# Kiteretsu77/This_and_That_VDM

Hardware: AMD Instinct MI355X
Metric: denoise-steps/sec (14-frame 256x448 VGL, 25 steps) (higher is better)
Workload: dtype bf16; 1 GPU; VGL denoise step: GestureNet ControlNet + spatio-temporal UNet + per-frame CFG + Euler, latent 14x4x32x56, CFG batch 2, 78 context tokens, heads (5,10,20,20); mode=vgl, requests_per_gpu=1, parallelism=1 independent request(s), one per GPU; RCCL weight broadcast at start-up only, hipgraph=True, finite_output=True, spatial_self_attention=bf16, weights_identical_on_all_ranks=True

## Files before the change

### this_and_that_vdm_amd/csrc/attention.hip

```cpp
#include <stdlib.h>
#include <type_traits>
#include "common.h"

#ifndef TT_ATTN_PIPE_SGB
#define TT_ATTN_PIPE_SGB 1
#endif

namespace {

struct AttnP {
  const char* q; long ldq;
  const char* k; long ldk;
  const char* vt; long ldvt;
  char* out; long ldo;
  int nseq, lq, heads;
  int mask, lk, k_seq_stride, v_seq_stride, frames, ctx_batches, batch0;
  int k_rows_total;
  long vt_cols_total;
  unsigned k_bytes, vt_bytes;
  float scale_log2e;
  const char* qx; long ldqx; const char* wq; long ldwq; const float* bq; int qc; float ln_eps;
  unsigned qx_bytes, wq_bytes;
  int v_rows;
};

constexpr int QB = 128;
constexpr int KB = 64;

__device__ __forceinline__ float fast_exp2(float x) { return __builtin_amdgcn_exp2f(x); }

struct Bid3 { int x, y, z; };
#ifndef TT_ATTN_QP_HEADFAST
#define TT_ATTN_QP_HEADFAST 1
#endif
template <bool HEADFAST = false>
__device__ __forceinline__ Bid3 xcd_remap3() {
  const int gx = gridDim.x, gy = gridDim.y;
  const int nwg = gx * gy * (int)gridDim.z;
  int bid = (int)blockIdx.x + gx * ((int)blockIdx.y + gy * (int)blockIdx.z);
  const int q = nwg >> 3, r = nwg & 7, xcd = bid & 7, idx = bid >> 3;
  bid = (xcd < r ? xcd * (q + 1) : r * (q + 1) + (xcd - r) * q) + idx;
  Bid3 o;
  if constexpr (HEADFAST) {
    o.y = bid % gy;
    const int t = bid / gy;
    o.x = t % gx;
    o.z = t / gx;
  } else {
    o.x = bid % gx;
    const int t = bid / gx;
    o.y = t % gy;
    o.z = t / gy;
  }
  return o;
}


__device__ __forceinline__ int key_perm(int l31) { return 16 * ((l31 >> 2) & 1) + (l31 & 3) + 4 * (l31 >> 3); }

template <int QES, int D>
__device__ __forceinline__ void load_q_frags(const AttnP& p, int seq, int head, int qrow, bool qok, int hi, uint4 (&qf)[D * QES / 32]) {
  const char* qp = p.q + (((long)seq * p.lq + (qok ? qrow : 0)) * p.ldq + head * D) * QES;
#pragma unroll
  for (int n = 0; n < D * QES / 32; ++n) qf[n] = qok ? *(const uint4*)(qp + (n * 2 + hi) * 16) : make_uint4(0, 0, 0, 0);
}

__device__ __forceinline__ void vr_read_addrs(int lane, unsigned lds_base, unsigned (&out)[2]) {
  const int gi = lane & 15, gg = lane >> 4, r2 = gi >> 2;
  const int base = ((gg & 1) * 2 + ((gi & 3) >> 1)) ^ ((gi >> 3) & 1);
#pragma unroll
  for (int half = 0; half < 2; ++half)
    out[half] = lds_base + (gg >> 1) * 2048 + r2 * 128 + half * 512 + ((base ^ (half << 1)) << 4) + (gi & 1) * 8;
}

template <int EB, int D, bool VR, int DH = D>
struct KvStage {
  static constexpr int EPC = 16 / EB;
  static constexpr int KCPR = D / EPC, VCPR = VR ? D / EPC : KB / EPC;
  static_assert(DH <= D && DH % EPC == 0, "whole chunks of the head");
  static constexpr int K_BYTES = KB * D * EB, V_BYTES = D * KB * EB, STAGE = K_BYTES + V_BYTES;
  static constexpr int KPT = (KB * KCPR) / 256, VPT = ((VR ? KB : D) * VCPR) / 256;
  static_assert(KPT * 4096 == K_BYTES && VPT * 4096 == V_BYTES, "the staged pieces cover each tile exactly");
  static constexpr int INV = (int)0x80000000;
  static_assert(KPT >= 1 && VPT >= 1, "tile smaller than the block");
  const AttnP& p;
  char* const ring;
  const __amdgpu_buffer_rsrc_t rk, rv;
  int kvo[KPT], kr[KPT], vvo[VPT], vc[VPT];
  const int k_rows_left;
  const long v_cols_left;
  __device__ __forceinline__ KvStage(const AttnP& p_, char* smem, int tid, int wid, int head, int kbase, int vbase)
      : p(p_), ring(smem + wid * 1024),
        rk(__builtin_amdgcn_make_buffer_rsrc((void*)p_.k, 0, p_.k_bytes, 0x00020000)),
        rv(__builtin_amdgcn_make_buffer_rsrc((void*)p_.vt, 0, p_.vt_bytes, 0x00020000)),
        k_rows_left(p_.k_rows_total - kbase), v_cols_left(p_.vt_cols_total - vbase) {
#pragma unroll
    for (int i = 0; i < KPT; ++i) {
      const int slot = i * 256 + tid;
      const int r = slot / KCPR, c = (slot % KCPR) ^ tile_swz<KCPR>(r);
      kr[i] = r;
      kvo[i] = (int)((((long)kbase + r) * p.ldk + head * DH + c * EPC) * EB);
      if (DH != D && c * EPC >= DH) kvo[i] = INV;
    }
#pragma unroll
    for (int i = 0; i < VPT; ++i) {
      const int slot = i * 256 + tid;
      const int r = slot / VCPR, c = (slot % VCPR) ^ tile_swz<VCPR>(r);
      if constexpr (VR) {
        vc[i] = r;
        vvo[i] = (int)((((long)vbase + r) * p.ldvt + head * DH + c * EPC) * EB);
        if (DH != D && c * EPC >= DH) vvo[i] = INV;
      } else {
        vc[i] = c * EPC;
        vvo[i] = (int)(((long)(head * DH + r) * p.ldvt + vbase + c * EPC) * EB);
        if (DH != D && r >= DH) vvo[i] = INV;
      }
    }
  }
  __device__ __forceinline__ void stage(int buf, int tile) const {
    const int j0 = tile * KB;
    char* lk_ = ring + buf * STAGE;
    char* lv_ = ring + buf * STAGE + K_BYTES;
    const int soff_k = __builtin_amdgcn_readfirstlane((int)((long)j0 * p.ldk * EB));
    const int soff_v = VR ? __builtin_amdgcn_readfirstlane((int)((long)j0 * p.ldvt * EB)) : j0 * EB;
    const bool edge = j0 + KB > k_rows_left || j0 + KB > v_cols_left;
#pragma unroll
    for (int i = 0; i < KPT; ++i) {
      int v = kvo[i];
      if (edge && j0 + kr[i] >= k_rows_left) v = INV;
      __builtin_amdgcn_raw_ptr_buffer_load_lds(rk, (__attribute__((address_space(3))) void*)(lk_ + i * 4096), 16, v, soff_k, 0, 0);
    }
#pragma unroll
    for (int i = 0; i < VPT; ++i) {
      int v = vvo[i];
      if (edge && j0 + vc[i] >= v_cols_left) v = INV;
      __builtin_amdgcn_raw_ptr_buffer_load_lds(rv, (__attribute__((address_space(3))) void*)(lv_ + i * 4096), 16, v, soff_v, 0, 0);
    }
  }
};

template <typename F>
__device__ __forceinline__ void for_each_tile(int ntiles, int lk, F&& tile) {
  const bool ragged = (lk % KB) != 0;
  const int full = ragged ? ntiles - 1 : ntiles;
  int t = 0;
  for (; t + 1 < full; t += 2) {
    tile(t, std::integral_constant<int, 0>{}, std::false_type{});
    tile(t + 1, std::integral_constant<int, 1>{}, std::false_type{});
  }
  if (t < full) {
    tile(t, std::integral_constant<int, 0>{}, std::false_type{});
    if (ragged) tile(t + 1, std::integral_constant<int, 1>{}, std::true_type{});
  } else if (ragged) {
    tile(t, std::integral_constant<int, 0>{}, std::true_type{});
  }
}

__device__ __forceinline__ void mask_ragged(f32x16_t (&s)[2], int t, int hi, int lk) {
  const int j0 = t * KB;
#pragma unroll
  for (int kb = 0; kb < 2; ++kb)
#pragma unroll
    for (int r = 0; r < 16; ++r) {
      const int j = j0 + kb * 32 + hi * 16 + r;
      if (j >= lk) s[kb][r] = -INFINITY;
    }
}

template <int NO, bool WITH_OX = false>
__device__ __forceinline__ void softmax_rescale(const f32x16_t (&s)[2], float scale_log2e, float& m_run, float& l_run, f32x16_t (&o)[NO],
                                                f32x16_t* ox = nullptr) {
  float mx = s[0][0];
#pragma unroll
  for (int kb = 0; kb < 2; ++kb)
#pragma unroll
    for (int r = 0; r < 16; ++r) mx = fmaxf(mx, s[kb][r]);
  mx = fmaxf(mx, __shfl_xor(mx, 32));
  const float m_new = fmaxf(m_run, mx * scale_log2e);
  const float alpha = fast_exp2(m_run - m_new);
  l_run *= alpha;
#pragma unroll
  for (int i = 0; i < NO; ++i)
#pragma unroll
    for (int r = 0; r < 16; ++r) { o[i][r] *= alpha; if constexpr (WITH_OX) ox[i][r] *= alpha; }
  m_run = m_new;
}

template <typename Tag, int D, int DO = D, int NO = D / 32>
__device__ __forceinline__ void attn_store_rows(const AttnP& p, char* smem, const f32x16_t (&o)[NO], float l_run, int wid, int lane,
                                                int seq, int head, int qblk, int qstride, int qcls) {
  static_assert(NO * 32 >= DO && NO * 32 <= D && (DO * Elem<Tag>::ES) % 16 == 0, "accumulators cover the stored columns");
  typedef typename Elem<Tag>::quad_t quad_t;
  constexpr int ES = Elem<Tag>::ES;
  const int l31 = lane & 31, hi = lane >> 5;
  const float l_tot = l_run + __shfl_xor(l_run, 32);
  const float inv = l_tot > 0.f ? 1.0f / l_tot : 0.f;
  __syncthreads();
  constexpr int ROWB_O = D * ES, CPR_O = ROWB_O / 16;
  char* strip = smem + wid * (32 * ROWB_O);
#pragma unroll
  for (int db = 0; db < NO; ++db)
#pragma unroll
    for (int g = 0; g < 4; ++g) {
      const int byte = (db * 32 + 8 * g + 4 * hi) * ES;
      const float v4[4] = {o[db][g * 4] * inv, o[db][g * 4 + 1] * inv, o[db][g * 4 + 2] * inv, o[db][g * 4 + 3] * inv};
      *(quad_t*)(strip + l31 * ROWB_O + (((byte >> 4) ^ (l31 & (CPR_O - 1))) << 4) + (byte & 15)) = f32_to_quad<Tag>(v4);
    }
  constexpr int RPP = 64 / CPR_O;
  const int oc = lane % CPR_O, orow = lane / CPR_O;
#pragma unroll
  for (int pass = 0; pass < 32 / RPP; ++pass) {
    const int r = pass * RPP + orow;
    const uint4 v = *(const uint4*)(strip + r * ROWB_O + ((oc ^ (r & (CPR_O - 1))) << 4));
    const int qr = (qblk * QB + wid * 32 + r) * qstride + qcls;
    if (qr < p.lq && (DO == D || oc * 16 < DO * ES)) *(uint4*)(p.out + (((long)seq * p.lq + qr) * p.ldo + head * DO) * ES + oc * 16) = v;
  }
}

template <typename Tag, int D, int MASK, bool QP = false, bool VR = false, bool SP = false>
__global__ __launch_bounds__(256, (D == 64 && Elem<Tag>::ES == 2) ? 2 : 1) void attn_kernel(const AttnP p) {
  static_assert(!VR || (D == 64 && Elem<Tag>::ES == 2 && MASK == 0 && !QP), "row-major V: spatial self-attention, head dimension 64, 16-bit storage");
  static_assert(!SP || (Elem<Tag>::ES == 4 && !QP && !VR), "split products: the fp32-storage kernel");
  kernarg_touch<sizeof(AttnP)>();
  extern __shared__ __attribute__((aligned(16))) char smem[];
  constexpr int ES = Elem<Tag>::ES, EPC = Elem<Tag>::EPC;
  typedef KvStage<ES, D, VR> Stage;
  constexpr int KCPR = Stage::KCPR, VCPR = Stage::VCPR, K_BYTES = Stage::K_BYTES, STAGE = Stage::STAGE;
  constexpr int DS = KCPR / 2, DB = D / 32;
  constexpr int PH = 16 / EPC;

  const int tid = threadIdx.x, lane = tid & 63;
  const int wid = __builtin_amdgcn_readfirstlane(tid >> 6);
  const int l31 = lane & 31, hi = lane >> 5;
  const Bid3 blk = xcd_remap3<QP && TT_ATTN_QP_HEADFAST>();
  const int head = blk.y, seq = blk.z;
  const char* zero = (const char*)tt_zero_page;

  const int qstride = MASK == 2 ? p.ctx_batches : 1;
  const int qcls = MASK == 2 ? blk.x % qstride : 0;
  const int qblk = MASK == 2 ? blk.x / qstride : blk.x;
  int kbase, vbase;
  if (MASK == 0) { kbase = seq * p.k_seq_stride; vbase = seq * p.v_seq_stride; }
  else {
    const int b = p.batch0 + seq / p.frames;
    const int ctx = MASK == 1 ? b : (int)(((long)b * p.lq + qcls) % p.ctx_batches);
    kbase = ctx * p.k_seq_stride; vbase = ctx * p.v_seq_stride;
  }
  const int ntiles = (p.lk + KB - 1) / KB;

  const int qrow = (qblk * QB + wid * 32 + l31) * qstride + qcls;
  const bool qok = qrow < p.lq;
  uint4 qf[DS];
  if constexpr (!QP) {
    load_q_frags<ES, D>(p, seq, head, qrow, qok, hi, qf);
  } else {
    static_assert(!QP || (D == 64 && ES == 2 && MASK != 0), "fused query projection: cross-attention, head dimension 64, 16-bit storage");
    constexpr int QSLAB = QB * 128 + 64 * 128, QNST = 3;
    constexpr int QINV = (int)0x80000000;
    const __amdgpu_buffer_rsrc_t rx = __builtin_amdgcn_make_buffer_rsrc((void*)p.qx, 0, p.qx_bytes, 0x00020000);
    const __amdgpu_buffer_rsrc_t rwq = __builtin_amdgcn_make_buffer_rsrc((void*)p.wq, 0, p.wq_bytes, 0x00020000);
    int xo[4], wo[2];
#pragma unroll
    for (int i = 0; i < 4; ++i) {
      const int slot = i * 256 + tid, r = slot >> 3, c = (slot & 7) ^ tile_swz<8>(r);
      const int qr = (qblk * QB + r) * qstride + qcls;
      xo[i] = qr < p.lq ? (int)((((long)seq * p.lq + qr) * p.ldqx + c * 8) * 2) : QINV;
    }
#pragma unroll
    for (int i = 0; i < 2; ++i) {
      const int slot = i * 256 + tid, r = slot >> 3, c = (slot & 7) ^ tile_swz<8>(r);
      wo[i] = (int)((((long)head * 64 + r) * p.ldwq + c * 8) * 2);
    }
    const int nslab = p.qc >> 6;
    auto qstage = [&](int s) {
      char* dst = smem + (s % QNST) * QSLAB + wid * 1024;
      const int soff = __builtin_amdgcn_readfirstlane(s * 128);
      const bool ok = s < nslab;
#pragma unroll
      for (int i = 0; i < 4; ++i)
        __builtin_amdgcn_raw_ptr_buffer_load_lds(rx, (__attribute__((address_space(3))) void*)(dst + i * 4096), 16, ok ? xo[i] : QINV, soff, 0, 0);
#pragma unroll
      for (int i = 0; i < 2; ++i)
        __builtin_amdgcn_raw_ptr_buffer_load_lds(rwq, (__attribute__((address_space(3))) void*)(dst + QB * 128 + i * 4096), 16, ok ? wo[i] : QINV, soff, 0, 0);
    };
    f32x16_t qa[2];
#pragma unroll
    for (int j = 0; j < 2; ++j)
#pragma unroll
      for (int r = 0; r < 16; ++r) qa[j][r] = 0.f;
    float ls = 0.f, lq2 = 0.f;
    const unsigned qbase = lds_addr(smem);
    const int xr = wid * 32 + l31;
    unsigned xa[4], wa[4];
#pragma unroll
    for (int ks = 0; ks < 4; ++ks) {
      xa[ks] = tile_off<8>(xr, ks * 2 + hi);
      wa[ks] = QB * 128 + tile_off<8>(l31, ks * 2 + hi);
    }
    qstage(0); qstage(1);
    for (int s = 0; s < nslab; ++s) {
      asm volatile("s_waitcnt vmcnt(6)" ::: "memory");
      __syncthreads();
      qstage(s + 2);
      const unsigned sb = qbase + (s % QNST) * QSLAB;
      raw_u32x4_t xf[4], wf[2][4];
#pragma unroll
      for (int ks = 0; ks < 4; ++ks) {
        xf[ks] = lds_read16_raw(sb + xa[ks]);
        wf[0][ks] = lds_read16_raw(sb + wa[ks]);
        wf[1][ks] = lds_read16_raw_off<4096>(sb + wa[ks]);
      }
      lds_wait<0>();
#pragma unroll
      for (int ks = 0; ks < 4; ++ks) {
        ln_stat<Tag>(xf[ks], ls, lq2);
#pragma unroll
        for (int j = 0; j < 2; ++j)
          qa[j] = Cvt<Tag>::mfma32(make_uint4(wf[j][ks].x, wf[j][ks].y, wf[j][ks].z, wf[j][ks].w),
                                   make_uint4(xf[ks].x, xf[ks].y, xf[ks].z, xf[ks].w), qa[j]);
      }
      __builtin_amdgcn_sched_barrier(0);
    }
    asm volatile("s_waitcnt vmcnt(0)" ::: "memory");
    __syncthreads();
    const float inv_c = 1.0f / (float)p.qc;
    const float sm = (ls + __shfl_xor(ls, 32)) * inv_c, sq = (lq2 + __shfl_xor(lq2, 32)) * inv_c;
    const float rs = rsqrtf(fmaxf(sq - sm * sm, 0.f) + p.ln_eps);
#pragma unroll
    for (int ds = 0; ds < DS; ++ds) {
      const int j = ds >> 1, t = ds & 1;
      const float4 b0 = *(const float4*)(p.bq + head * 64 + 32 * j + 8 * (2 * t) + 4 * hi);
      const float4 b1 = *(const float4*)(p.bq + head * 64 + 32 * j + 8 * (2 * t + 1) + 4 * hi);
      const float v[8] = {fmaf(qa[j][(2 * t) * 4], rs, b0.x), fmaf(qa[j][(2 * t) * 4 + 1], rs, b0.y), fmaf(qa[j][(2 * t) * 4 + 2], rs, b0.z),
                          fmaf(qa[j][(2 * t) * 4 + 3], rs, b0.w), fmaf(qa[j][(2 * t + 1) * 4], rs, b1.x), fmaf(qa[j][(2 * t + 1) * 4 + 1], rs, b1.y),
                          fmaf(qa[j][(2 * t + 1) * 4 + 2], rs, b1.z), fmaf(qa[j][(2 * t + 1) * 4 + 3], rs, b1.w)};
      qf[ds] = qok ? pack8<Tag>(v) : make_uint4(0, 0, 0, 0);
    }
  }

  const Stage kv(p, smem, tid, wid, head, kbase, vbase);

  f32x16_t o[DB];
#pragma unroll
  for (int i = 0; i < DB; ++i)
#pragma unroll
    for (int r = 0; r < 16; ++r) o[i][r] = 0.f;
  float m_run = -1e30f, l_run = 0.f;
  f32x16_t ox[SP ? DB : 1];
  uint4 qh[SP ? DS / 2 : 1], ql[SP ? DS / 2 : 1];
  if constexpr (SP) {
#pragma unroll
    for (int i = 0; i < DB; ++i)
#pragma unroll
      for (int r = 0; r < 16; ++r) ox[i][r] = 0.f;
#pragma unroll
    for (int i = 0; i < DS / 2; ++i) {
      uint2 h0, l0, h1, l1;
      split_f16x4(qf[2 * i].x, qf[2 * i].y, qf[2 * i].z, qf[2 * i].w, h0, l0);
      split_f16x4(qf[2 * i + 1].x, qf[2 * i + 1].y, qf[2 * i + 1].z, qf[2 * i + 1].w, h1, l1);
      qh[i] = make_uint4(h0.x, h0.y, h1.x, h1.y); ql[i] = make_uint4(l0.x, l0.y, l1.x, l1.y);
    }
  }

  const int pi = key_perm(l31);

  const unsigned lds_base = lds_addr(smem);
  constexpr bool PRE = D == 64 && ES == 2;
  unsigned kaddr[PRE ? 2 : 1][PRE ? DS : 1], vaddr[PRE ? DB : 1][PRE ? 2 * PH : 1];
  if constexpr (PRE) {
#pragma unroll
    for (int kb = 0; kb < 2; ++kb)
#pragma unroll
      for (int ds = 0; ds < DS; ++ds) kaddr[kb][ds] = lds_base + tile_off<KCPR>(kb * 32 + pi, ds * 2 + hi);
#pragma unroll
    for (int db = 0; db < DB; ++db)
#pragma unroll
      for (int k = 0; k < 2 * PH; ++k) vaddr[db][k] = lds_base + tile_off<VCPR>(db * 32 + l31, (k / PH) * (32 / EPC) + hi * PH + k % PH);
  }
  unsigned vr_addr[2] = {0u, 0u};
  if constexpr (VR) vr_read_addrs(lane, lds_base, vr_addr);
  auto k_addr = [&](int kb, int ds) -> unsigned {
    if constexpr (PRE) return kaddr[kb][ds]; else return lds_base + tile_off<KCPR>(kb * 32 + pi, ds * 2 + hi);
  };
  auto v_addr = [&](int db, int k) -> unsigned {
    if constexpr (PRE) return vaddr[db][k]; else return lds_base + tile_off<VCPR>(db * 32 + l31, (k / PH) * (32 / EPC) + hi * PH + k % PH);
  };

  constexpr int NBK = DS / 2;
  constexpr int NBV = (DB / 2) * PH;
  static_assert(DS % 2 == 0 && DB % 2 == 0, "fragment batches of four");
  auto tile = [&](int t, auto buf_tag, auto mask_tag) {
    constexpr int BUF = decltype(buf_tag)::value;
    constexpr bool MASKED = decltype(mask_tag)::value;
    constexpr int KOFF = BUF * STAGE, VOFF = BUF * STAGE + K_BYTES;
    asm volatile("s_waitcnt vmcnt(0)" ::: "memory");
    __syncthreads();
    if (t + 1 < ntiles) kv.stage(BUF ^ 1, t + 1);
    raw_u32x4_t fa[4], fb[4];
    auto read_k = [&](int i, raw_u32x4_t (&f)[4]) {
#pragma unroll
      for (int j = 0; j < 4; ++j) f[j] = lds_read16_raw_off<KOFF>(k_addr(j & 1, 2 * i + (j >> 1)));
    };
    auto read_v = [&](int i, raw_u32x4_t (&f)[4]) {
#pragma unroll
      for (int j = 0; j < 4; ++j) f[j] = lds_read16_raw_off<VOFF>(v_addr(2 * (i / PH) + (j & 1), 2 * (i % PH) + (j >> 1)));
    };
    raw_u32x2_t ga[8], gb[8];
    auto read_vr = [&](auto i_tag, raw_u32x2_t (&f)[8]) {
      constexpr int I = decltype(i_tag)::value;
      auto one = [&](auto j_tag) {
        constexpr int J = decltype(j_tag)::value;
        constexpr int db = 2 * (I / PH) + (J & 1), k = 2 * (I % PH) + (J >> 1), kb = k / PH, h = k % PH;
        constexpr int off = VOFF + kb * 4096 + h * 1024 + ((db ^ h) << 6);
        f[2 * J] = lds_read8_tr_off<off>(vr_addr[0]);
        f[2 * J + 1] = lds_read8_tr_off<off>(vr_addr[1]);
      };
      one(std::integral_constant<int, 0>{}); one(std::integral_constant<int, 1>{});
      one(std::integral_constant<int, 2>{}); one(std::integral_constant<int, 3>{});
    };
    f32x16_t s[2], sx[SP ? 2 : 1];
#pragma unroll
    for (int kb = 0; kb < 2; ++kb)
#pragma unroll
      for (int r = 0; r < 16; ++r) { s[kb][r] = 0.f; if constexpr (SP) sx[kb][r] = 0.f; }
    read_k(0, fa);
    read_k(1, fb);
#pragma unroll
    for (int i = 0; i < NBK; ++i) {
      if (i + 1 < NBK) lds_wait<4>(); else lds_wait<0>();
      const raw_u32x4_t (&f)[4] = (i & 1) ? fb : fa;
      if constexpr (SP) {
#pragma unroll
        for (int kb = 0; kb < 2; ++kb) {
          uint2 h0, l0, h1, l1;
          split_f16x4(f[kb].x, f[kb].y, f[kb].z, f[kb].w, h0, l0);
          split_f16x4(f[kb + 2].x, f[kb + 2].y, f[kb + 2].z, f[kb + 2].w, h1, l1);
          const uint4 kh = make_uint4(h0.x, h0.y, h1.x, h1.y), kl = make_uint4(l0.x, l0.y, l1.x, l1.y);
          sx[kb] = Cvt<f16_tag>::mfma32(kl, qh[i], sx[kb]);
          s[kb] = Cvt<f16_tag>::mfma32(kh, qh[i], s[kb]);
          sx[kb] = Cvt<f16_tag>::mfma32(kh, ql[i], sx[kb]);
        }
      } else {
#pragma unroll
      for (int j = 0; j < 4; ++j)
        s[j & 1] = Cvt<Tag>::mfma32(make_uint4(f[j].x, f[j].y, f[j].z, f[j].w), qf[2 * i + (j >> 1)], s[j & 1]);
      }
      __builtin_amdgcn_sched_barrier(0);
      if (i + 2 < NBK) { if (i & 1) read_k(i + 2, fb); else read_k(i + 2, fa); }
    }
    if constexpr (VR) {
      read_vr(std::integral_constant<int, 0>{}, ga);
      read_vr(std::integral_constant<int, 1>{}, gb);
    } else if constexpr (!SP) {
      read_v(0, fa);
      if constexpr (NBV > 1) read_v(1, fb);
    }
    if constexpr (SP) {
#pragma unroll
      for (int kb = 0; kb < 2; ++kb)
#pragma unroll
        for (int r = 0; r < 16; ++r) s[kb][r] = fmaf(sx[kb][r], 32.0f, s[kb][r] * 65536.0f);
    }
    if constexpr (MASKED) mask_ragged(s, t, hi, p.lk);
    constexpr float PSUM_OK = 16384.0f;
    float psum = 0.f;
    uint4 pf[2][PH];
    uint2 ph2[SP ? 2 : 1][SP ? PH : 1], pl2[SP ? 2 : 1][SP ? PH : 1];
    auto exponentiate = [&](float m_ref) {
      psum = 0.f;
#pragma unroll
      for (int kb = 0; kb < 2; ++kb)
#pragma unroll
        for (int h = 0; h < PH; ++h) {
          float e[EPC];
#pragma unroll
          for (int r = 0; r < EPC; ++r) { e[r] = fast_exp2(fmaf(s[kb][h * EPC + r], p.scale_log2e, -m_ref)); psum += e[r]; }
          pf[kb][h] = pack_chunk<Tag>(e);
        }
    };
    exponentiate(m_run);
    if (__any(!(psum <= PSUM_OK))) {
      softmax_rescale<DB, SP>(s, p.scale_log2e, m_run, l_run, o, ox);
      exponentiate(m_run);
    }
    l_run += psum;
    if constexpr (SP) {
#pragma unroll
      for (int kb = 0; kb < 2; ++kb)
#pragma unroll
        for (int h = 0; h < PH; ++h) split_f16x4(pf[kb][h].x, pf[kb][h].y, pf[kb][h].z, pf[kb][h].w, ph2[kb][h], pl2[kb][h]);
      __builtin_amdgcn_sched_barrier(0);
      read_v(0, fa);
      if constexpr (NBV > 1) read_v(1, fb);
    }
    if constexpr (VR) {
#pragma unroll
      for (int i = 0; i < NBV; ++i) {
        if (i + 1 < NBV) lds_wait<8>(); else lds_wait<0>();
        const raw_u32x2_t (&f)[8] = (i & 1) ? gb : ga;
#pragma unroll
        for (int j = 0; j < 4; ++j) {
          const int db = 2 * (i / PH) + (j & 1), k = 2 * (i % PH) + (j >> 1);
          o[db] = Cvt<Tag>::mfma32(make_uint4(f[2 * j].x, f[2 * j].y, f[2 * j + 1].x, f[2 * j + 1].y), pf[k / PH][k % PH], o[db]);
        }
        __builtin_amdgcn_sched_barrier(0);
      }
    } else {
#pragma unroll
    for (int i = 0; i < NBV; ++i) {
      if (i + 1 < NBV) lds_wait<4>(); else lds_wait<0>();
      const raw_u32x4_t (&f)[4] = (i & 1) ? fb : fa;
      if constexpr (SP) {
        const int k0 = 2 * (i % PH), kb = k0 / PH, h0 = k0 % PH;
        const uint4 ph = make_uint4(ph2[kb][h0].x, ph2[kb][h0].y, ph2[kb][h0 + 1].x, ph2[kb][h0 + 1].y);
        const uint4 pl = make_uint4(pl2[kb][h0].x, pl2[kb][h0].y, pl2[kb][h0 + 1].x, pl2[kb][h0 + 1].y);
#pragma unroll
        for (int jd = 0; jd < 2; ++jd) {
          const int db = 2 * (i / PH) + jd;
          uint2 vh0, vl0, vh1, vl1;
          split_f16x4(f[jd].x, f[jd].y, f[jd].z, f[jd].w, vh0, vl0);
          split_f16x4(f[jd + 2].x, f[jd + 2].y, f[jd + 2].z, f[jd + 2].w, vh1, vl1);
          const uint4 vh = make_uint4(vh0.x, vh0.y, vh1.x, vh1.y), vl = make_uint4(vl0.x, vl0.y, vl1.x, vl1.y);
          ox[db] = Cvt<f16_tag>::mfma32(vl, ph, ox[db]);
          o[db] = Cvt<f16_tag>::mfma32(vh, ph, o[db]);
          ox[db] = Cvt<f16_tag>::mfma32(vh, pl, ox[db]);
        }
      } else {
#pragma unroll
      for (int j = 0; j < 4; ++j) {
        const int db = 2 * (i / PH) + (j & 1), k = 2 * (i % PH) + (j >> 1);
        o[db] = Cvt<Tag>::mfma32(make_uint4(f[j].x, f[j].y, f[j].z, f[j].w), pf[k / PH][k % PH], o[db]);
      }
      }
      __builtin_amdgcn_sched_barrier(0);
      if (i + 2 < NBV) { if (i & 1) read_v(i + 2, fb); else read_v(i + 2, fa); }
    }
    }
  };

  kv.stage(0, 0);
  for_each_tile(ntiles, p.lk, tile);
  if constexpr (SP) {
#pragma unroll
    for (int i = 0; i < DB; ++i)
#pragma unroll
      for (int r = 0; r < 16; ++r) o[i][r] = fmaf(ox[i][r], 32.0f, o[i][r] * 65536.0f);
  }
  static_assert(4 * 32 * D * ES <= 2 * STAGE, "output strips do not fit the K/V ring");
  attn_store_rows<Tag, D>(p, smem, o, l_run, wid, lane, seq, head, qblk, qstride, qcls);
}

template <typename Tag>
__global__ __launch_bounds__(256, 2) void attn_pipe_kernel(const AttnP p) {
  static_assert(Elem<Tag>::ES == 2, "16-bit storage");
  kernarg_touch<sizeof(AttnP)>();
  extern __shared__ __attribute__((aligned(16))) char smem[];
  constexpr int D = 64, ES = 2, EPC = 8, CPR = 8;
  constexpr int K_BYTES = KB * D * ES, V_BYTES = KB * D * ES, PT = (KB * CPR) / 256;
  const int tid = threadIdx.x, lane = tid & 63;
  const int wid = __builtin_amdgcn_readfirstlane(tid >> 6);
  const int l31 = lane & 31, hi = lane >> 5;
  const Bid3 blk = xcd_remap3<false>();
  const int head = blk.y, seq = blk.z;
  const int kbase = seq * p.k_seq_stride, vbase = seq * p.v_seq_stride;
  const int nt = p.lk / KB;

  const int qrow = blk.x * QB + wid * 32 + l31;
  const bool qok = qrow < p.lq;
  uint4 qf[4];
  load_q_frags<ES, D>(p, seq, head, qrow, qok, hi, qf);
  const __amdgpu_buffer_rsrc_t rk = __builtin_amdgcn_make_buffer_rsrc((void*)p.k, 0, p.k_bytes, 0x00020000);
  const __amdgpu_buffer_rsrc_t rv = __builtin_amdgcn_make_buffer_rsrc((void*)p.vt, 0, p.vt_bytes, 0x00020000);
  int kvo[PT], vvo[PT];
#pragma unroll
  for (int i = 0; i < PT; ++i) {
    const int slot = i * 256 + tid;
    const int r = slot / CPR, c = (slot % CPR) ^ tile_swz<CPR>(r);
    kvo[i] = (int)((((long)kbase + r) * p.ldk + head * D + c * EPC) * ES);
    vvo[i] = (int)((((long)vbase + r) * p.ldvt + head * D + c * EPC) * ES);
  }
  auto stage_k = [&](int buf, int tile) {
    char* l_ = smem + buf * K_BYTES + wid * 1024;
    const int soff = __builtin_amdgcn_readfirstlane((int)((long)tile * KB * p.ldk * ES));
#pragma unroll
    for (int i = 0; i < PT; ++i)
      __builtin_amdgcn_raw_ptr_buffer_load_lds(rk, (__attribute__((address_space(3))) void*)(l_ + i * 4096), 16, kvo[i], soff, 0, 0);
  };
  auto stage_v = [&](int buf, int tile) {
    char* l_ = smem + 2 * K_BYTES + buf * V_BYTES + wid * 1024;
    const int soff = __builtin_amdgcn_readfirstlane((int)((long)tile * KB * p.ldvt * ES));
#pragma unroll
    for (int i = 0; i < PT; ++i)
      __builtin_amdgcn_raw_ptr_buffer_load_lds(rv, (__attribute__((address_space(3))) void*)(l_ + i * 4096), 16, vvo[i], soff, 0, 0);
  };

  f32x16_t o[2];
#pragma unroll
  for (int i = 0; i < 2; ++i)
#pragma unroll
    for (int r = 0; r < 16; ++r) o[i][r] = 0.f;
  float m_run = -1e30f, l_run = 0.f;
  uint4 P[4];
#pragma unroll
  for (int c = 0; c < 4; ++c) P[c] = make_uint4(0, 0, 0, 0);

  const int pi = key_perm(l31);
  const unsigned lds_base = lds_addr(smem);
  unsigned kaddr[4];
#pragma unroll
  for (int ds = 0; ds < 4; ++ds) kaddr[ds] = lds_base + tile_off<CPR>(pi, ds * 2 + hi);
  unsigned vr_addr[2];
  vr_read_addrs(lane, lds_base, vr_addr);
  constexpr float PSUM_OK = 16384.0f;

  auto tile = [&](int t, auto buf_tag, auto pv_tag) {
    constexpr int BUF = decltype(buf_tag)::value;
    constexpr bool HAS_PV = decltype(pv_tag)::value;
    constexpr int KOFF = BUF * K_BYTES, VOFF = 2 * K_BYTES + (BUF ^ 1) * V_BYTES;
    asm volatile("s_waitcnt vmcnt(0)" ::: "memory");
    __syncthreads();
    if (t + 1 < nt) stage_k(BUF ^ 1, t + 1);
    stage_v(BUF, t);
    raw_u32x4_t x[2], y[2];
    auto request_k = [&](auto n_tag, raw_u32x4_t (&f)[2]) {
      constexpr int N = decltype(n_tag)::value;
      f[0] = lds_read16_raw_off<KOFF + (N >> 1) * 4096>(kaddr[2 * (N & 1)]);
      f[1] = lds_read16_raw_off<KOFF + (N >> 1) * 4096>(kaddr[2 * (N & 1) + 1]);
    };
    auto request_v = [&](auto m_tag, raw_u32x4_t (&f)[2]) {
      constexpr int M = decltype(m_tag)::value;
      constexpr int kb = M / 2, h = M % 2;
      auto one = [&](auto db_tag) {
        constexpr int db = decltype(db_tag)::value;
        constexpr int off = VOFF + kb * 4096 + h * 1024 + ((db ^ h) << 6);
        const raw_u32x2_t lo = lds_read8_tr_off<off>(vr_addr[0]), hi2 = lds_read8_tr_off<off>(vr_addr[1]);
        f[db] = (raw_u32x4_t){lo.x, lo.y, hi2.x, hi2.y};
      };
      one(std::integral_constant<int, 0>{}); one(std::integral_constant<int, 1>{});
    };
    f32x16_t sc[2];
#pragma unroll
    for (int kb = 0; kb < 2; ++kb)
#pragma unroll
      for (int r = 0; r < 16; ++r) sc[kb][r] = 0.f;
    auto multiply_k = [&](int n, const raw_u32x4_t (&f)[2]) {
      const int kb = n >> 1, ds = 2 * (n & 1);
      sc[kb] = Cvt<Tag>::mfma32(make_uint4(f[0].x, f[0].y, f[0].z, f[0].w), qf[ds], sc[kb]);
      sc[kb] = Cvt<Tag>::mfma32(make_uint4(f[1].x, f[1].y, f[1].z, f[1].w), qf[ds + 1], sc[kb]);
    };
    auto multiply_v = [&](int m, const raw_u32x4_t (&f)[2]) {
#pragma unroll
      for (int db = 0; db < 2; ++db) o[db] = Cvt<Tag>::mfma32(make_uint4(f[db].x, f[db].y, f[db].z, f[db].w), P[m], o[db]);
    };
    float psum = 0.f;
    uint4 Pn[4];
    float e[8];
    auto exp_part = [&](int c, int part) {
      const int kb = c >> 1, h = c & 1;
#pragma unroll
      for (int r = part * 4; r < part * 4 + 4; ++r) { e[r] = fast_exp2(fmaf(sc[kb][h * 8 + r], p.scale_log2e, -m_run)); psum += e[r]; }
      if (part) Pn[c] = pack_chunk<Tag>(e);
    };
    auto exp_chunk = [&](int c) { exp_part(c, 0); exp_part(c, 1); };
    auto beside = [&](auto valu_tag) {
#if TT_ATTN_PIPE_SGB
      constexpr int VALU = decltype(valu_tag)::value;
      __builtin_amdgcn_sched_group_barrier(0x008, 1, 0); __builtin_amdgcn_sched_group_barrier(0x002, VALU, 0);
      __builtin_amdgcn_sched_group_barrier(0x008, 1, 0); __builtin_amdgcn_sched_group_barrier(0x002, VALU, 0);
#endif
    };
    request_k(std::integral_constant<int, 0>{}, x);
    request_k(std::integral_constant<int, 1>{}, y);
    lds_wait<2>(); multiply_k(0, x); __builtin_amdgcn_sched_barrier(0);
    request_k(std::integral_constant<int, 2>{}, x);
    lds_wait<2>(); multiply_k(1, y); __builtin_amdgcn_sched_barrier(0);
    request_k(std::integral_constant<int, 3>{}, y);
    lds_wait<2>(); multiply_k(2, x); exp_chunk(0); beside(std::integral_constant<int, 14>{}); __builtin_amdgcn_sched_barrier(0);
    if constexpr (HAS_PV) request_v(std::integral_constant<int, 0>{}, x);
    if constexpr (HAS_PV) lds_wait<4>(); else lds_wait<0>();
    multiply_k(3, y); exp_chunk(1); beside(std::integral_constant<int, 14>{}); __builtin_amdgcn_sched_barrier(0);
    if constexpr (HAS_PV) {
      request_v(std::integral_constant<int, 1>{}, y);
      lds_wait<4>(); multiply_v(0, x); exp_part(2, 0); beside(std::integral_constant<int, 7>{}); __builtin_amdgcn_sched_barrier(0);
      request_v(std::integral_constant<int, 2>{}, x);
      lds_wait<4>(); multiply_v(1, y); exp_part(2, 1); beside(std::integral_constant<int, 7>{}); __builtin_amdgcn_sched_barrier(0);
      request_v(std::integral_constant<int, 3>{}, y);
      lds_wait<4>(); multiply_v(2, x); exp_part(3, 0); beside(std::integral_constant<int, 7>{}); __builtin_amdgcn_sched_barrier(0);
      lds_wait<0>(); multiply_v(3, y); exp_part(3, 1); beside(std::integral_constant<int, 7>{}); __builtin_amdgcn_sched_barrier(0);
    } else {
      exp_chunk(2); exp_chunk(3);
    }
    if (__any(!(psum <= PSUM_OK))) {
      softmax_rescale<2>(sc, p.scale_log2e, m_run, l_run, o);
      psum = 0.f;
      exp_chunk(0); exp_chunk(1); exp_chunk(2); exp_chunk(3);
    }
    l_run += psum;
#pragma unroll
    for (int c = 0; c < 4; ++c) P[c] = Pn[c];
  };
  typedef std::integral_constant<int, 0> B0;
  typedef std::integral_constant<int, 1> B1;

  stage_k(0, 0);
  tile(0, B0{}, std::false_type{});
  {
    int t = 1;
    for (; t + 1 < nt; t += 2) {
      tile(t, B1{}, std::true_type{});
      tile(t + 1, B0{}, std::true_type{});
    }
    if (t < nt) tile(t, B1{}, std::true_type{});
  }
  auto final_pv = [&](auto buf_tag) {
    constexpr int BUF = decltype(buf_tag)::value;
    constexpr int VOFF = 2 * K_BYTES + BUF * V_BYTES;
    asm volatile("s_waitcnt vmcnt(0)" ::: "memory");
    __syncthreads();
    raw_u32x2_t g[16];
    auto one = [&](auto n_tag) {
      constexpr int N = decltype(n_tag)::value, k = N >> 1, db = N & 1, kb = k / 2, h = k % 2;
      constexpr int off = VOFF + kb * 4096 + h * 1024 + ((db ^ h) << 6);
      g[2 * N] = lds_read8_tr_off<off>(vr_addr[0]);
      g[2 * N + 1] = lds_read8_tr_off<off>(vr_addr[1]);
    };
    one(std::integral_constant<int, 0>{}); one(std::integral_constant<int, 1>{}); one(std::integral_constant<int, 2>{}); one(std::integral_constant<int, 3>{});
    one(std::integral_constant<int, 4>{}); one(std::integral_constant<int, 5>{}); one(std::integral_constant<int, 6>{}); one(std::integral_constant<int, 7>{});
    lds_wait<0>();
#pragma unroll
    for (int n = 0; n < 8; ++n) {
      const int k = n >> 1, db = n & 1;
      o[db] = Cvt<Tag>::mfma32(make_uint4(g[2 * n].x, g[2 * n].y, g[2 * n + 1].x, g[2 * n + 1].y), P[k], o[db]);
    }
    __builtin_amdgcn_sched_barrier(0);
  };
  if ((nt - 1) & 1) final_pv(B1{}); else final_pv(B0{});

  attn_store_rows<Tag, D>(p, smem, o, l_run, wid, lane, seq, head, blk.x, 1, 0);
}

typedef long fp8x8_t;
template <typename Tag, int D>
__global__ __launch_bounds__(256, 2) void attn8_kernel(const AttnP p) {
  kernarg_touch<sizeof(AttnP)>();
  extern __shared__ __attribute__((aligned(16))) char smem[];
  typedef KvStage<1, D, false> Stage;
  constexpr int KCPR = Stage::KCPR, VCPR = Stage::VCPR, K_BYTES = Stage::K_BYTES, STAGE = Stage::STAGE;
  constexpr int JJ = D / 32, DB = D / 32;
  const int tid = threadIdx.x, lane = tid & 63;
  const int wid = __builtin_amdgcn_readfirstlane(tid >> 6);
  const int l31 = lane & 31, hi = lane >> 5;
  const Bid3 blk = xcd_remap3();
  const int head = blk.y, seq = blk.z, qblk = blk.x;
  const int kbase = seq * p.k_seq_stride, vbase = seq * p.v_seq_stride;
  const int ntiles = (p.lk + KB - 1) / KB;
  const int qrow = qblk * QB + wid * 32 + l31;
  const bool qok = qrow < p.lq;
  uint4 qf[JJ];
  load_q_frags<1, D>(p, seq, head, qrow, qok, hi, qf);
  const Stage kv(p, smem, tid, wid, head, kbase, vbase);
  f32x16_t o[DB];
#pragma unroll
  for (int i = 0; i < DB; ++i)
#pragma unroll
    for (int r = 0; r < 16; ++r) o[i][r] = 0.f;
  float m_run = -1e30f, l_run = 0.f;
  const int pi = key_perm(l31);
  const unsigned lds_base = lds_addr(smem);
  unsigned kaddr[2][JJ], vaddr[DB][2];
#pragma unroll
  for (int kb = 0; kb < 2; ++kb)
#pragma unroll
    for (int jj = 0; jj < JJ; ++jj) kaddr[kb][jj] = lds_base + tile_off<KCPR>(kb * 32 + pi, 2 * jj + hi);
#pragma unroll
  for (int db = 0; db < DB; ++db)
#pragma unroll
    for (int kb = 0; kb < 2; ++kb) vaddr[db][kb] = lds_base + tile_off<VCPR>(db * 32 + l31, 2 * kb + hi);
  typedef int v8i_t __attribute__((ext_vector_type(8)));
  auto mfma8 = [](const v8i_t& a, const v8i_t& b, f32x16_t c) {
    return __builtin_amdgcn_mfma_scale_f32_32x32x64_f8f6f4(a, b, c, 0, 0, 0, 0x7f7f7f7f, 0, 0x7f7f7f7f);
  };
  auto pack8 = [](const raw_u32x4_t& lo, const raw_u32x4_t& hi_) {
    return (v8i_t){(int)lo.x, (int)lo.y, (int)lo.z, (int)lo.w, (int)hi_.x, (int)hi_.y, (int)hi_.z, (int)hi_.w};
  };
  static_assert(JJ % 2 == 0, "two 16-byte chunks per K = 64 MFMA");
  v8i_t qv[JJ / 2];
#pragma unroll
  for (int m = 0; m < JJ / 2; ++m)
    qv[m] = (v8i_t){(int)qf[2 * m].x, (int)qf[2 * m].y, (int)qf[2 * m].z, (int)qf[2 * m].w,
                    (int)qf[2 * m + 1].x, (int)qf[2 * m + 1].y, (int)qf[2 * m + 1].z, (int)qf[2 * m + 1].w};
  auto tile = [&](int t, auto buf_tag, auto mask_tag) {
    constexpr int BUF = decltype(buf_tag)::value;
    constexpr bool MASKED = decltype(mask_tag)::value;
    constexpr int KOFF = BUF * STAGE, VOFF = BUF * STAGE + K_BYTES;
    asm volatile("s_waitcnt vmcnt(0)" ::: "memory");
    __syncthreads();
    if (t + 1 < ntiles) kv.stage(BUF ^ 1, t + 1);
    raw_u32x4_t kf[2][JJ], vf[DB][2];
#pragma unroll
    for (int jj = 0; jj < JJ; ++jj)
#pragma unroll
      for (int kb = 0; kb < 2; ++kb) kf[kb][jj] = lds_read16_raw_off<KOFF>(kaddr[kb][jj]);
    f32x16_t s[2];
#pragma unroll
    for (int kb = 0; kb < 2; ++kb)
#pragma unroll
      for (int r = 0; r < 16; ++r) s[kb][r] = 0.f;
    lds_wait<0>();
#pragma unroll
    for (int m = 0; m < JJ / 2; ++m)
#pragma unroll
      for (int kb = 0; kb < 2; ++kb)
        s[kb] = mfma8(pack8(kf[kb][2 * m], kf[kb][2 * m + 1]), qv[m], s[kb]);
    __builtin_amdgcn_sched_barrier(0);
#pragma unroll
    for (int kb = 0; kb < 2; ++kb)
#pragma unroll
      for (int db = 0; db < DB; ++db) vf[db][kb] = lds_read16_raw_off<VOFF>(vaddr[db][kb]);
    if constexpr (MASKED) mask_ragged(s, t, hi, p.lk);
    constexpr float PSUM_OK = 448.0f, P_LOG2 = 3.0f;
    float psum = 0.f;
    unsigned pf[2][2][2];
    auto exponentiate = [&](float shift) {
      psum = 0.f;
#pragma unroll
      for (int kb = 0; kb < 2; ++kb)
#pragma unroll
        for (int h = 0; h < 2; ++h) {
          float e[8];
#pragma unroll
          for (int r = 0; r < 8; ++r) { e[r] = fast_exp2(fmaf(s[kb][h * 8 + r], p.scale_log2e, shift)); psum += e[r]; }
          int w0 = 0, w1 = 0;
          w0 = __builtin_amdgcn_cvt_pk_fp8_f32(e[0], e[1], w0, false);
          w0 = __builtin_amdgcn_cvt_pk_fp8_f32(e[2], e[3], w0, true);
          w1 = __builtin_amdgcn_cvt_pk_fp8_f32(e[4], e[5], w1, false);
          w1 = __builtin_amdgcn_cvt_pk_fp8_f32(e[6], e[7], w1, true);
          pf[kb][h][0] = (unsigned)w0; pf[kb][h][1] = (unsigned)w1;
        }
    };
    exponentiate(P_LOG2 - m_run);
    if (__any(!(psum <= PSUM_OK))) {
      softmax_rescale<DB>(s, p.scale_log2e, m_run, l_run, o);
      exponentiate(P_LOG2 - m_run);
// ... 631 lines not shown
```

Before: 35.96 denoise-steps/s.

## Prefetch first K/V tiles during fused Q-projection and preload bias early

In the fused Q-projection attention path, the first two K/V tiles are now staged into ring slots while the Q-projection slab loop is still running, instead of only after it finishes. The tile stride is widened so those stages fit between the Q slabs, and the waitcnt logic is adjusted so the first tile waits for only part of the outstanding loads. The bq bias values are also loaded up front with inline asm so their latency overlaps the projection. This hides the K/V load latency at the start of attention, at the cost of more fragile vmcnt bookkeeping and a larger LDS layout.

```diff
diff --git a/this_and_that_vdm_amd/csrc/attention.hip b/this_and_that_vdm_amd/csrc/attention.hip
--- a/this_and_that_vdm_amd/csrc/attention.hip
+++ b/this_and_that_vdm_amd/csrc/attention.hip
@@ -32,6 +32,9 @@
 struct Bid3 { int x, y, z; };
 #ifndef TT_ATTN_QP_HEADFAST
 #define TT_ATTN_QP_HEADFAST 1
+#endif
+#ifndef TT_ATTN_QP_EARLY
+#define TT_ATTN_QP_EARLY 1
 #endif
 template <bool HEADFAST = false>
 __device__ __forceinline__ Bid3 xcd_remap3() {
@@ -56,6 +59,13 @@
 }
 
 
+template <int OFF> __device__ __forceinline__ raw_f32x4_t global_read16_raw_off(const void* ptr) {
+  static_assert(OFF >= 0 && OFF < 4096, "offset");
+  raw_f32x4_t v;
+  asm volatile("global_load_dwordx4 %0, %1, off offset:%2" : "=v"(v) : "v"(ptr), "n"(OFF));
+  return v;
+}
+
 __device__ __forceinline__ int key_perm(int l31) { return 16 * ((l31 >> 2) & 1) + (l31 & 3) + 4 * (l31 >> 3); }
 
 template <int QES, int D>
@@ -73,12 +83,13 @@
     out[half] = lds_base + (gg >> 1) * 2048 + r2 * 128 + half * 512 + ((base ^ (half << 1)) << 4) + (gi & 1) * 8;
 }
 
-template <int EB, int D, bool VR, int DH = D>
+template <int EB, int D, bool VR, int DH = D, int STRIDE = 0>
 struct KvStage {
   static constexpr int EPC = 16 / EB;
   static constexpr int KCPR = D / EPC, VCPR = VR ? D / EPC : KB / EPC;
   static_assert(DH <= D && DH % EPC == 0, "whole chunks of the head");
-  static constexpr int K_BYTES = KB * D * EB, V_BYTES = D * KB * EB, STAGE = K_BYTES + V_BYTES;
+  static constexpr int K_BYTES = KB * D * EB, V_BYTES = D * KB * EB, STAGE = K_BYTES + V_BYTES, BSTRIDE = STRIDE ? STRIDE : STAGE;
+  static_assert(BSTRIDE >= STAGE, "stages overlap");
   static constexpr int KPT = (KB * KCPR) / 256, VPT = ((VR ? KB : D) * VCPR) / 256;
   static_assert(KPT * 4096 == K_BYTES && VPT * 4096 == V_BYTES, "the staged pieces cover each tile exactly");
   static constexpr int INV = (int)0x80000000;
@@ -119,8 +130,8 @@
   }
   __device__ __forceinline__ void stage(int buf, int tile) const {
     const int j0 = tile * KB;
-    char* lk_ = ring + buf * STAGE;
-    char* lv_ = ring + buf * STAGE + K_BYTES;
+    char* lk_ = ring + buf * BSTRIDE;
+    char* lv_ = ring + buf * BSTRIDE + K_BYTES;
     const int soff_k = __builtin_amdgcn_readfirstlane((int)((long)j0 * p.ldk * EB));
     const int soff_v = VR ? __builtin_amdgcn_readfirstlane((int)((long)j0 * p.ldvt * EB)) : j0 * EB;
     const bool edge = j0 + KB > k_rows_left || j0 + KB > v_cols_left;
@@ -224,8 +235,9 @@
   kernarg_touch<sizeof(AttnP)>();
   extern __shared__ __attribute__((aligned(16))) char smem[];
   constexpr int ES = Elem<Tag>::ES, EPC = Elem<Tag>::EPC;
-  typedef KvStage<ES, D, VR> Stage;
-  constexpr int KCPR = Stage::KCPR, VCPR = Stage::VCPR, K_BYTES = Stage::K_BYTES, STAGE = Stage::STAGE;
+  constexpr bool QPE = QP && TT_ATTN_QP_EARLY != 0;
+  typedef KvStage<ES, D, VR, D, QPE ? QB * 128 + 64 * 128 : 0> Stage;
+  constexpr int KCPR = Stage::KCPR, VCPR = Stage::VCPR, K_BYTES = Stage::K_BYTES, STAGE = Stage::STAGE, TSTRIDE = Stage::BSTRIDE;
   constexpr int DS = KCPR / 2, DB = D / 32;
   constexpr int PH = 16 / EPC;
 
@@ -297,6 +309,76 @@
       xa[ks] = tile_off<8>(xr, ks * 2 + hi);
       wa[ks] = QB * 128 + tile_off<8>(l31, ks * 2 + hi);
     }
+    if constexpr (QPE) {
+      static_assert(Stage::KPT + Stage::VPT == 4 && Stage::STAGE <= QSLAB && 2 * QSLAB + Stage::STAGE <= QNST * QSLAB, "tile stages in ring slots 0 and 1");
+      raw_f32x4_t bqe[DS][2];
+      const float* bqp = p.bq + head * 64 + 4 * hi;
+      static_assert(DS == 4, "eight float4 of bq per lane");
+      bqe[0][0] = global_read16_raw_off<0>(bqp); bqe[0][1] = global_read16_raw_off<32>(bqp);
+      bqe[1][0] = global_read16_raw_off<64>(bqp); bqe[1][1] = global_read16_raw_off<96>(bqp);
+      bqe[2][0] = global_read16_raw_off<128>(bqp); bqe[2][1] = global_read16_raw_off<160>(bqp);
+      bqe[3][0] = global_read16_raw_off<192>(bqp); bqe[3][1] = global_read16_raw_off<224>(bqp);
+      __builtin_amdgcn_sched_barrier(0);
+      const Stage kvq(p, smem, tid, wid, head, kbase, vbase);
+      const int rot = (QNST - nslab % QNST) % QNST;
+      auto qround = [&](int r, int slot) {
+        if (r < nslab) {
+          char* dst = smem + slot * QSLAB + wid * 1024;
+          const int soff = __builtin_amdgcn_readfirstlane(r * 128);
+#pragma unroll
+          for (int i = 0; i < 4; ++i)
+            __builtin_amdgcn_raw_ptr_buffer_load_lds(rx, (__attribute__((address_space(3))) void*)(dst + i * 4096), 16, xo[i], soff, 0, 0);
+#pragma unroll
+          for (int i = 0; i < 2; ++i)
+            __builtin_amdgcn_raw_ptr_buffer_load_lds(rwq, (__attribute__((address_space(3))) void*)(dst + QB * 128 + i * 4096), 16, wo[i], soff, 0, 0);
+        } else if (r - nslab < ntiles) {
+          kvq.stage(r - nslab, r - nslab);
+        }
+      };
+      int slot = rot;
+      qround(0, rot); qround(1, rot == 2 ? 0 : rot + 1);
+      for (int s = 0; s < nslab; ++s) {
+        if (s + 1 < nslab) asm volatile("s_waitcnt vmcnt(6)" ::: "memory");
+        else asm volatile("s_waitcnt vmcnt(4)" ::: "memory");
+        __builtin_amdgcn_s_barrier(); asm volatile("" ::: "memory");
+        qround(s + 2, slot == 0 ? 2 : slot - 1);
+        const unsigned sb = qbase + slot * QSLAB;
+        slot = slot == 2 ? 0 : slot + 1;
+        raw_u32x4_t xf[4], wf[2][4];
+#pragma unroll
+        for (int ks = 0; ks < 4; ++ks) {
+          xf[ks] = lds_read16_raw(sb + xa[ks]);
+          wf[0][ks] = lds_read16_raw(sb + wa[ks]);
+          wf[1][ks] = lds_read16_raw_off<4096>(sb + wa[ks]);
+        }
+#pragma unroll
+        for (int half = 0; half < 2; ++half) {
+          if (half == 0) lds_wait<6>(); else lds_wait<0>();
+#pragma unroll
+          for (int ks = 2 * half; ks < 2 * half + 2; ++ks) {
+            ln_stat<Tag>(xf[ks], ls, lq2);
+#pragma unroll
+            for (int j = 0; j < 2; ++j)
+              qa[j] = Cvt<Tag>::mfma32(make_uint4(wf[j][ks].x, wf[j][ks].y, wf[j][ks].z, wf[j][ks].w),
+                                       make_uint4(xf[ks].x, xf[ks].y, xf[ks].z, xf[ks].w), qa[j]);
+          }
+        }
+        __builtin_amdgcn_sched_barrier(0);
+      }
+      const float inv_c = 1.0f / (float)p.qc;
+      const float sm = (ls + __shfl_xor(ls, 32)) * inv_c, sq = (lq2 + __shfl_xor(lq2, 32)) * inv_c;
+      const float rs = rsqrtf(fmaxf(sq - sm * sm, 0.f) + p.ln_eps);
+      asm volatile("" : "+v"(bqe[0][0]), "+v"(bqe[0][1]), "+v"(bqe[1][0]), "+v"(bqe[1][1]), "+v"(bqe[2][0]), "+v"(bqe[2][1]), "+v"(bqe[3][0]), "+v"(bqe[3][1]));
+#pragma unroll
+      for (int ds = 0; ds < DS; ++ds) {
+        const int j = ds >> 1, t = ds & 1;
+        const raw_f32x4_t b0 = bqe[ds][0], b1 = bqe[ds][1];
+        const float v[8] = {fmaf(qa[j][(2 * t) * 4], rs, b0.x), fmaf(qa[j][(2 * t) * 4 + 1], rs, b0.y), fmaf(qa[j][(2 * t) * 4 + 2], rs, b0.z),
+                            fmaf(qa[j][(2 * t) * 4 + 3], rs, b0.w), fmaf(qa[j][(2 * t + 1) * 4], rs, b1.x), fmaf(qa[j][(2 * t + 1) * 4 + 1], rs, b1.y),
+                            fmaf(qa[j][(2 * t + 1) * 4 + 2], rs, b1.z), fmaf(qa[j][(2 * t + 1) * 4 + 3], rs, b1.w)};
+        qf[ds] = qok ? pack8<Tag>(v) : make_uint4(0, 0, 0, 0);
+      }
+    } else {
     qstage(0); qstage(1);
     for (int s = 0; s < nslab; ++s) {
       asm volatile("s_waitcnt vmcnt(6)" ::: "memory");
@@ -336,6 +418,7 @@
                           fmaf(qa[j][(2 * t + 1) * 4 + 2], rs, b1.z), fmaf(qa[j][(2 * t + 1) * 4 + 3], rs, b1.w)};
       qf[ds] = qok ? pack8<Tag>(v) : make_uint4(0, 0, 0, 0);
     }
+    }
   }
 
   const Stage kv(p, smem, tid, wid, head, kbase, vbase);
@@ -392,10 +475,17 @@
   auto tile = [&](int t, auto buf_tag, auto mask_tag) {
     constexpr int BUF = decltype(buf_tag)::value;
     constexpr bool MASKED = decltype(mask_tag)::value;
-    constexpr int KOFF = BUF * STAGE, VOFF = BUF * STAGE + K_BYTES;
+    constexpr int KOFF = BUF * TSTRIDE, VOFF = BUF * TSTRIDE + K_BYTES;
+    if constexpr (QPE) {
+      if (t == 0 && ntiles >= 2) asm volatile("s_waitcnt vmcnt(4)" ::: "memory");
+      else asm volatile("s_waitcnt vmcnt(0)" ::: "memory");
+      __builtin_amdgcn_s_barrier(); asm volatile("" ::: "memory");
+      if (t >= 1 && t + 1 < ntiles) kv.stage(BUF ^ 1, t + 1);
+    } else {
     asm volatile("s_waitcnt vmcnt(0)" ::: "memory");
     __syncthreads();
     if (t + 1 < ntiles) kv.stage(BUF ^ 1, t + 1);
+    }
     raw_u32x4_t fa[4], fb[4];
     auto read_k = [&](int i, raw_u32x4_t (&f)[4]) {
 #pragma unroll
@@ -538,7 +628,7 @@
     }
   };
 
-  kv.stage(0, 0);
+  if constexpr (!QPE) kv.stage(0, 0);
   for_each_tile(ntiles, p.lk, tile);
   if constexpr (SP) {
 #pragma unroll
```

Result: no change. 36.03 denoise-steps/s (median of 6 runs) (+0.2%).
